# pyannote/pyannote-audio

Hardware: NVIDIA H100
Metric: audio-hours/sec (RTF) community-1 diarization, 16kHz mono, 1/2/4/8 H100 (higher is better)
Workload: dtype f16 tensor-core trunk (f32 accumulate) + split-f16x3 tensor-core segmentation (f32-level accuracy) + f64 clustering

## Files before the change

### pyannote_audio_b200/csrc/emb_conv.cu

```cuda
#include "common.cuh"
#include "emb.cuh"
#include "tc_common.cuh"

namespace b200 {

constexpr int kWgThreads = 288;
constexpr int kTileM = 128;
constexpr int kRowHalo = 8;
constexpr int kMaxSlots = 16;

template <int N, bool WIDE = false, int MH = 1>
__device__ __forceinline__ void conv_epilogue(const float* acc, const ConvParams& p, size_t row, int w0) {
  const int lane = threadIdx.x & 31;
  const int c0 = 2 * (lane & 3) + (WIDE ? (int)blockIdx.y * N : 0);
#pragma unroll
  for (int m = 0; m < MH; ++m)
#pragma unroll
  for (int i = 0; i < 2; ++i) {
    const int w = w0 + 64 * m + ((threadIdx.x >> 5) & 3) * 16 + (lane >> 2) + 8 * i;
    if (w >= p.W_out) continue;
    const size_t pix = (row * p.W_out + w) * (size_t)(WIDE ? p.C_out : N);
    __half2 res[N / 8];
    if (N <= 128 && p.residual) {
#pragma unroll
// ... 28 lines not shown
  const int wt = blockIdx.x % p.tiles_w;
  const int bh = blockIdx.x / p.tiles_w;
  const int cchunks = p.C_in / CK;

  if (threadIdx.x == 0) {
    for (uint32_t s = 0; s < p.nstages; ++s) { mbar_init(bar_full + 8 * s, 1); mbar_init(bar_empty + 8 * s, 2); }
    asm volatile("fence.mbarrier_init.release.cluster;" ::: "memory");
  }
  __syncthreads();

  if (warp == 8) {
    if ((threadIdx.x & 31) == 0) {
      prefetch_tensormap(&tmA);
      prefetch_tensormap(&tmB);
      const int h = bh % p.H_out, b = bh / p.H_out;
      const int w_base = wt * kTileM * p.stride - p.pad, h_base = h * p.stride - p.pad;
      uint32_t stage = 0, phase = 0;
      for (int kh = 0; kh < p.taps_h; ++kh)
        for (int kw = 0; kw < p.taps_w; ++kw)
          for (int cc = 0; cc < cchunks; ++cc) {
            mbar_wait(bar_empty + 8 * stage, phase ^ 1);
            mbar_expect_tx(bar_full + 8 * stage, p.a_tx + p.b_bytes);
            const uint32_t sa = stage0 + stage * stage_bytes;
            tma_load_4d(&tmA, bar_full + 8 * stage, sa, cc * CK, w_base + kw, h_base + kh, b);
            tma_load_3d(&tmB, bar_full + 8 * stage, sa + p.a_bytes, cc * CK, WIDE ? (int)blockIdx.y * N : 0,
                        kh * p.taps_w + kw);
            if (++stage == p.nstages) { stage = 0; phase ^= 1; }
          }
    }
    return;
  }

  const int wg = warp >> 2;
  constexpr uint32_t row_bytes = CK * 2;
  float acc[N / 2];
#pragma unroll
  for (int i = 0; i < N / 2; ++i) acc[i] = 0.f;
  const int kblocks = p.taps_h * p.taps_w * cchunks;
  uint32_t stage = 0, phase = 0, prev = 0;
  for (int kb = 0; kb < kblocks; ++kb) {
    mbar_wait(bar_full + 8 * stage, phase);
    const uint32_t st = stage0 + stage * stage_bytes;
    const uint32_t sa = st + (uint32_t)wg * 64u * row_bytes, sb = st + p.a_bytes;
    wg_fence();
    const uint64_t ad = wg_desc(sa, row_bytes), bd = wg_desc(sb, row_bytes);
#pragma unroll
    for (int k = 0; k < CK / 16; ++k) Wgmma<N>::mma(acc, ad + 2 * k, bd + 2 * k);
    wg_commit();
    wg_wait<1>();
    if (kb > 0 && (threadIdx.x & 127) == 0) mbar_arrive(bar_empty + 8 * prev);
    prev = stage;
    if (++stage == p.nstages) { stage = 0; phase ^= 1; }
  }
  wg_wait<0>();
  conv_epilogue<N, WIDE>(acc, p, (size_t)bh, wt * kTileM + wg * 64);
}

template <int N>
__device__ __forceinline__ void row_taps_c32(float (&acc)[2][N / 2], uint32_t sa, uint32_t wts) {
  constexpr uint32_t row_bytes = 64;
  const int warp = threadIdx.x >> 5, lane = threadIdx.x & 31;
#pragma unroll
  for (int kw = 0; kw < 3; ++kw) {
    uint32_t af[2][2][4];
#pragma unroll
    for (int m = 0; m < 2; ++m)
#pragma unroll
      for (int k = 0; k < 2; ++k) {
        const uint32_t row = (uint32_t)(m * 64 + (warp & 3) * 16 + (lane & 15) + kw);
        const uint32_t chunk = (uint32_t)(2 * k + (lane >> 4)) ^ ((row >> 1) & 3u);
        ldsm_x4(af[m][k], sa + row * row_bytes + chunk * 16u);
      }
    wg_fence();
    const uint64_t bd = wg_desc(wts + kw * N * row_bytes, row_bytes);
#pragma unroll
    for (int k = 0; k < 2; ++k)
#pragma unroll
      for (int m = 0; m < 2; ++m) WgmmaRS<N>::mma(acc[m], af[m][k], bd + 2 * k);
    wg_commit();
    wg_wait<0>();
  }
}

template <int N, int CK>
__global__ void __launch_bounds__(kWgThreads, N == 32 ? 2 : 1)
conv_row_kernel(const __grid_constant__ CUtensorMap tmA, const __grid_constant__ CUtensorMap tmB, ConvParams p) {
  constexpr uint32_t row_bytes = CK * 2;
  constexpr uint32_t b_tap_bytes = N * row_bytes;
  extern __shared__ uint8_t smem_raw[];
  const uint32_t base = (smem_u32(smem_raw) + 1023u) & ~1023u;
  const uint32_t bar_w = base, bar_full = base + 8, bar_empty = base + 8 + 8 * kMaxSlots;
  const uint32_t wts = base + 1024;
  const uint32_t slot0 = wts + 9 * b_tap_bytes;
  const uint32_t nslots = p.nstages;
  const int warp = threadIdx.x >> 5;

  if (threadIdx.x == 0) {
    mbar_init(bar_w, 1);
    for (uint32_t s = 0; s < nslots; ++s) { mbar_init(bar_full + 8 * s, 1); mbar_init(bar_empty + 8 * s, 3); }
    asm volatile("fence.mbarrier_init.release.cluster;" ::: "memory");
  }
  __syncthreads();

  if (warp == 8) {
    if ((threadIdx.x & 31) == 0) {
      prefetch_tensormap(&tmA);
      prefetch_tensormap(&tmB);
      mbar_expect_tx(bar_w, 9 * b_tap_bytes);
      for (int kh = 0; kh < 3; ++kh) tma_load_3d(&tmB, bar_w, wts + 3 * kh * b_tap_bytes, 0, 0, 3 * kh);
      uint32_t s = 0;
      for (int u = blockIdx.x; u < p.num_tiles; u += gridDim.x) {
        const int wt = u % p.tiles_w, t = u / p.tiles_w;
        const int h0 = (t % p.bands) * p.band, b = t / p.bands;
        const int n = min(p.band, p.H_out - h0);
        for (int r = 0; r < n + 2; ++r, ++s) {
          const uint32_t slot = s % nslots;
          mbar_wait(bar_empty + 8 * slot, ((s / nslots) & 1) ^ 1);
          mbar_expect_tx(bar_full + 8 * slot, p.a_tx);
          tma_load_4d(&tmA, bar_full + 8 * slot, slot0 + slot * p.a_bytes, 0, wt * kTileM - 1, h0 - 1 + r, b);
        }
      }
    }
    return;
  }

  const int wg = __shfl_sync(0xffffffffu, warp >> 2, 0);
  mbar_wait(bar_w, 0);
  uint32_t s = 0;
  int item = 0;
  for (int u = blockIdx.x; u < p.num_tiles; u += gridDim.x) {
    const int wt = u % p.tiles_w, t = u / p.tiles_w;
    const int h0 = (t % p.bands) * p.band, b = t / p.bands;
    const int n = min(p.band, p.H_out - h0);
    for (int j = 0; j < n; ++j, ++item) {
      if ((item & 1) != wg) continue;
      float acc[2][N / 2];
#pragma unroll
      for (int m = 0; m < 2; ++m)
#pragma unroll
        for (int i = 0; i < N / 2; ++i) {
          acc[m][i] = 0.f;
          asm volatile("" : "+f"(acc[m][i]));
        }
#pragma unroll
      for (int kh = 0; kh < 3; ++kh) {
        const uint32_t q = s + j + kh, slot = q % nslots;
        mbar_wait(bar_full + 8 * slot, (q / nslots) & 1);
        const uint32_t sa = slot0 + slot * p.a_bytes;
        if constexpr (CK == 32) {
          row_taps_c32<N>(acc, sa, wts + 3 * kh * b_tap_bytes);
        } else {
          wg_fence();
#pragma unroll
          for (int kw = 0; kw < 3; ++kw) {
            const uint64_t bd = wg_desc(wts + (3 * kh + kw) * b_tap_bytes, row_bytes);
#pragma unroll
            for (int m = 0; m < 2; ++m) {
              const uint64_t ad = wg_desc(sa + (uint32_t)(m * 64 + kw) * row_bytes, row_bytes);
#pragma unroll
              for (int k = 0; k < CK / 16; ++k) Wgmma<N>::mma(acc[m], ad + 2 * k, bd + 2 * k);
            }
          }
          wg_commit();
        }
      }
      wg_wait<0>();
      if ((threadIdx.x & 127) == 0)
#pragma unroll
        for (int kh = 0; kh < 3; ++kh)
          mbar_arrive_n(bar_empty + 8 * ((s + j + kh) % nslots), 1 + (j == 0 ? 2 - kh : 0) + (j == n - 1 ? kh : 0));
      const size_t row = (size_t)b * p.H_out + h0 + j;
#pragma unroll
      for (int m = 0; m < 2; ++m) conv_epilogue<N>(acc[m], p, row, wt * kTileM + m * 64);
    }
    s += n + 2;
  }
}

struct BlockRowPlan {
  static constexpr uint32_t kTapBytes = 32 * 64;
  static constexpr uint32_t kSlotBytes = 9 * 1024;
  static constexpr uint32_t kInTx = (kTileM + kRowHalo) * 64;
  static constexpr uint32_t kInSlots = 4, kMidSlots = 4;
  static constexpr size_t kSmem = 2048 + 2 * 9 * kTapBytes + (kInSlots + kMidSlots) * kSlotBytes;
  static_assert(kInTx <= kSlotBytes && kSmem <= 113 * 1024, "block row plan");
};
constexpr int kStripW = kTileM - 2;

struct BlockParams {
  int H, W, tiles_w, band, bands, num_tiles;
  const float* bias1;
  const float* bias2;
  __half* out;
};

__device__ __forceinline__ void st_shared_u32(uint32_t a, uint32_t v) {
  asm volatile("st.shared.b32 [%0], %1;" ::"r"(a), "r"(v) : "memory");
}
__device__ __forceinline__ uint32_t ld_shared_u32(uint32_t a) {
  uint32_t v;
  asm volatile("ld.shared.b32 %0, [%1];" : "=r"(v) : "r"(a) : "memory");
  return v;
}
__device__ __forceinline__ uint32_t h2_bits(__half2 h) { return *reinterpret_cast<uint32_t*>(&h); }

__global__ void __launch_bounds__(kWgThreads, 2)
block_row_kernel(const __grid_constant__ CUtensorMap tmA, const __grid_constant__ CUtensorMap tmW1,
                 const __grid_constant__ CUtensorMap tmW2, BlockParams p) {
  using P = BlockRowPlan;
  constexpr uint32_t NI = P::kInSlots, NM = P::kMidSlots;
  extern __shared__ uint8_t smem_raw[];
  const uint32_t base = (smem_u32(smem_raw) + 1023u) & ~1023u;
  const uint32_t bar_w = base, in_full = base + 8, in_empty = in_full + 8 * NI;
  const uint32_t mid_full = in_empty + 8 * NI, mid_empty = mid_full + 8 * NM;
  const uint32_t w1 = base + 1024, w2 = w1 + 9 * P::kTapBytes;
  const uint32_t in0 = w2 + 9 * P::kTapBytes, mid0 = in0 + NI * P::kSlotBytes;
  const int warp = threadIdx.x >> 5, lane = threadIdx.x & 31;

  if (threadIdx.x == 0) {
    mbar_init(bar_w, 1);
    for (uint32_t s = 0; s < NI; ++s) { mbar_init(in_full + 8 * s, 1); mbar_init(in_empty + 8 * s, 4); }
    for (uint32_t s = 0; s < NM; ++s) { mbar_init(mid_full + 8 * s, 128); mbar_init(mid_empty + 8 * s, 3); }
    asm volatile("fence.mbarrier_init.release.cluster;" ::: "memory");
  }
  __syncthreads();

  if (warp == 8) {
    if (lane == 0) {
      prefetch_tensormap(&tmA);
      prefetch_tensormap(&tmW1);
      prefetch_tensormap(&tmW2);
      mbar_expect_tx(bar_w, 18 * P::kTapBytes);
      for (int kh = 0; kh < 3; ++kh) {
        tma_load_3d(&tmW1, bar_w, w1 + 3 * kh * P::kTapBytes, 0, 0, 3 * kh);
        tma_load_3d(&tmW2, bar_w, w2 + 3 * kh * P::kTapBytes, 0, 0, 3 * kh);
      }
      uint32_t s = 0;
      for (int u = blockIdx.x; u < p.num_tiles; u += gridDim.x) {
        const int wt = u % p.tiles_w, t = u / p.tiles_w;
        const int h0 = (t % p.bands) * p.band, b = t / p.bands;
        const int n = min(p.band, p.H - h0);
        for (int r = 0; r < n + 4; ++r, ++s) {
          const uint32_t slot = s % NI;
          mbar_wait(in_empty + 8 * slot, ((s / NI) & 1) ^ 1);
          mbar_expect_tx(in_full + 8 * slot, P::kInTx);
          tma_load_4d(&tmA, in_full + 8 * slot, in0 + slot * P::kSlotBytes, 0, wt * kStripW - 2, h0 - 2 + r, b);
        }
      }
    }
    return;
  }

  const int wg = __shfl_sync(0xffffffffu, warp >> 2, 0);
  const bool leader = (threadIdx.x & 127) == 0;
  const int c0 = 2 * (lane & 3);
  float2 bias[4];
#pragma unroll
  for (int j = 0; j < 4; ++j) bias[j] = __ldg(reinterpret_cast<const float2*>((wg ? p.bias2 : p.bias1) + 8 * j + c0));
  mbar_wait(bar_w, 0);
  uint32_t s = 0, mq = 0;
  for (int u = blockIdx.x; u < p.num_tiles; u += gridDim.x) {
    const int wt = u % p.tiles_w, t = u / p.tiles_w;
    const int h0 = (t % p.bands) * p.band, b = t / p.bands;
    const int n = min(p.band, p.H - h0);
    const int w0 = wt * kStripW;
    const int rows = wg == 0 ? n + 2 : n;
    for (int j = 0; j < rows; ++j) {
      float acc[2][16];
#pragma unroll
      for (int m = 0; m < 2; ++m)
#pragma unroll
        for (int i = 0; i < 16; ++i) {
          acc[m][i] = 0.f;
          asm volatile("" : "+f"(acc[m][i]));
        }
      if (wg == 0) {
#pragma unroll
        for (int kh = 0; kh < 3; ++kh) {
          const uint32_t q = s + j + kh, slot = q % NI;
          mbar_wait(in_full + 8 * slot, (q / NI) & 1);
          row_taps_c32<32>(acc, in0 + slot * P::kSlotBytes, w1 + 3 * kh * P::kTapBytes);
        }
        if (leader)
#pragma unroll
          for (int kh = 0; kh < 3; ++kh) {
            const int k = j + kh;
            const bool no_res = (k < 2 || k >= n + 2) && j == min(k, n + 1);
// ... 297 lines not shown
      for (int q = 0; q < 8; ++q) {
        const ulonglong2 w4 = wk[q];
        ffma2(acc2[2 * q], xk, w4.x);
        ffma2(acc2[2 * q + 1], xk, w4.y);
      }
    }
    __half2 o[16];
#pragma unroll
    for (int c = 0; c < 16; ++c) {
      float a0, a1;
      unpack2(acc2[c], a0, a1);
      o[c] = __floats2half2_rn(fmaxf(a0, 0.f), fmaxf(a1, 0.f));
    }
    uint4* op = reinterpret_cast<uint4*>(out + (((size_t)b * kMel + h) * T0 + t) * 32);
    const uint4* src = reinterpret_cast<const uint4*>(o);
#pragma unroll
    for (int i = 0; i < 4; ++i) op[i] = src[i];
  }
}

typedef CUresult (*PFN_encodeTiled)(CUtensorMap*, CUtensorMapDataType, cuuint32_t, void*, const cuuint64_t*,
                                    const cuuint64_t*, const cuuint32_t*, const cuuint32_t*, CUtensorMapInterleave,
                                    CUtensorMapSwizzle, CUtensorMapL2promotion, CUtensorMapFloatOOBfill);

static PFN_encodeTiled get_encode() {
  static PFN_encodeTiled fn = nullptr;
  if (!fn) {
    void* ptr = nullptr;
    cudaDriverEntryPointQueryResult qres;
    if (cudaGetDriverEntryPoint("cuTensorMapEncodeTiled", &ptr, cudaEnableDefault, &qres) == cudaSuccess &&
        qres == cudaDriverEntryPointSuccess)
      fn = reinterpret_cast<PFN_encodeTiled>(ptr);
  }
  return fn;
}

int encode_f16_map(CUtensorMap* tm, int rank, const void* ptr, const cuuint64_t* dims, const cuuint64_t* strides,
                   const cuuint32_t* box, const cuuint32_t* estr, CUtensorMapSwizzle swizzle, const char* what) {
  PFN_encodeTiled enc = get_encode();
  B200_CHECK(enc != nullptr, B200_ERR_CUDA, "cuTensorMapEncodeTiled not available from the driver");
  const cuuint32_t ones[5] = {1, 1, 1, 1, 1};
  CUresult r = enc(tm, CU_TENSOR_MAP_DATA_TYPE_FLOAT16, (cuuint32_t)rank, const_cast<void*>(ptr), dims, strides, box,
                   estr ? estr : ones, CU_TENSOR_MAP_INTERLEAVE_NONE, swizzle, CU_TENSOR_MAP_L2_PROMOTION_L2_256B,
                   CU_TENSOR_MAP_FLOAT_OOB_FILL_NONE);
  B200_CHECK(r == CUDA_SUCCESS, B200_ERR_CUDA, "cuTensorMapEncodeTiled(%s) failed: %d", what, (int)r);
  return B200_OK;
}

int conv_forward(const ConvLayer& L, const __half* in, const __half* residual, __half* out, int B, int H_in, int W_in,
                 int relu, int impl, int num_sms, cudaStream_t stream) {
  ConvParams p{};
  p.B = B; p.H_in = H_in; p.W_in = W_in; p.C_in = L.C_in; p.C_out = L.C_out;
  p.taps_h = L.ksize; p.taps_w = L.ksize; p.stride = L.stride; p.pad = L.ksize / 2;
  p.H_out = (H_in + 2 * p.pad - L.ksize) / L.stride + 1;
  p.W_out = (W_in + 2 * p.pad - L.ksize) / L.stride + 1;
  p.relu = relu; p.bias = L.bias; p.residual = residual; p.out = out;
  p.Ck = (L.C_in >= 64) ? 64 : 32;
  p.swizzle = (p.Ck == 64) ? 128 : 64;
  p.tiles_w = ceil_div(p.W_out, kTileM);
  p.num_tiles = B * p.H_out * p.tiles_w;
  B200_CHECK(L.C_in % p.Ck == 0 && (L.C_out == 32 || L.C_out == 64 || L.C_out == 128 ||
                                    (L.C_out % 256 == 0 && L.C_out <= 1024 && p.Ck == 64)),
             B200_ERR_STATE, "conv %d -> %d channels unsupported", L.C_in, L.C_out);
  const int n_tile = std::min(L.C_out, 256);
  B200_CHECK(impl >= 0 && impl <= 2, B200_ERR_INVALID,
             "conv_impl %d unknown (0 = CUDA cores, 1 = tensor cores, 2 = tensor cores, one weight tap per stage)", impl);

  if (impl == 0) {
    const size_t total = (size_t)B * p.H_out * p.W_out * (L.C_out / 8);
    conv_simt_kernel<<<(unsigned)((total + 255) / 256), 256, 0, stream>>>(in, L.w, p);
    B200_CUDA_OK(cudaGetLastError());
    return B200_OK;
  }

  const bool rows = impl == 1 && L.ksize == 3 && L.stride == 1 && L.C_in == p.Ck && L.C_out == L.C_in;
  const bool chunk_rows =
      impl == 1 && L.ksize == 3 && L.stride == 1 && L.C_out == L.C_in && (L.C_out == 128 || L.C_out == 256);
  p.a_rows = rows || chunk_rows ? kTileM + kRowHalo : kTileM;
  p.a_tx = p.a_rows * p.Ck * 2;
  p.a_bytes = (p.a_tx + 1023u) & ~1023u;
  size_t smem;
  int ctas = 0;
  if (rows) {
    const int per_sm = L.C_out == 32 ? 2 : 1;
    const size_t budget = per_sm == 2 ? 113u * 1024 : 227u * 1024;
    const size_t fixed = 2048 + (size_t)9 * L.C_out * p.Ck * 2;
    p.nstages = (uint32_t)std::min<size_t>(kMaxSlots, (budget - fixed) / p.a_bytes);
    B200_CHECK(p.nstages >= 6, B200_ERR_STATE, "conv %d -> %d: row ring too shallow", L.C_in, L.C_out);
    smem = fixed + (size_t)p.nstages * p.a_bytes;
    ctas = per_sm * num_sms;
    const int strips = B * p.tiles_w;
    const int nbands = std::min(p.H_out, ceil_div(ctas, strips));
    p.band = ceil_div(p.H_out, nbands);
    p.bands = ceil_div(p.H_out, p.band);
    p.num_tiles = strips * p.bands;
  } else if (chunk_rows) {
    p.band = L.C_out == 256 ? ChunkRowPlan<256>::kRows : ChunkRowPlan<128>::kRows;
    p.bands = ceil_div(p.H_out, p.band);
    p.num_tiles = B * p.bands * p.tiles_w;
    smem = L.C_out == 256 ? ChunkRowPlan<256>::kSmem : ChunkRowPlan<128>::kSmem;
    ctas = num_sms;
  } else {
    p.b_bytes = (uint32_t)(n_tile * p.Ck * 2);
    const uint32_t budget = n_tile == 256 ? 200u * 1024 : 100u * 1024;
    p.nstages = std::min(budget / (p.a_bytes + p.b_bytes), 8u);
    B200_CHECK(p.nstages >= 2, B200_ERR_STATE, "conv %d -> %d: shared memory plan too shallow", L.C_in, L.C_out);
    smem = 1024 + 1024 + (size_t)p.nstages * (p.a_bytes + p.b_bytes);
  }
  const CUtensorMapSwizzle swz = p.swizzle == 128 ? CU_TENSOR_MAP_SWIZZLE_128B : CU_TENSOR_MAP_SWIZZLE_64B;
  CUtensorMap tmA, tmB;
  int rc;
  {
    const cuuint64_t dims[4] = {(cuuint64_t)L.C_in, (cuuint64_t)W_in, (cuuint64_t)H_in, (cuuint64_t)B};
    const cuuint64_t strides[3] = {(cuuint64_t)L.C_in * 2, (cuuint64_t)W_in * L.C_in * 2,
                                   (cuuint64_t)H_in * W_in * L.C_in * 2};
    const cuuint32_t box[4] = {(cuuint32_t)p.Ck, (cuuint32_t)(p.a_rows * L.stride), 1, 1};
    const cuuint32_t estr[4] = {1, (cuuint32_t)L.stride, 1, 1};
    if ((rc = encode_f16_map(&tmA, 4, in, dims, strides, box, estr, swz, "A"))) return rc;
  }
  {
    const cuuint64_t dims[3] = {(cuuint64_t)L.C_in, (cuuint64_t)L.C_out, (cuuint64_t)(L.ksize * L.ksize)};
    const cuuint64_t strides[2] = {(cuuint64_t)L.C_in * 2, (cuuint64_t)L.C_out * L.C_in * 2};
    const cuuint32_t box[3] = {(cuuint32_t)p.Ck, (cuuint32_t)n_tile, rows ? 3u : 1u};
    if ((rc = encode_f16_map(&tmB, 3, L.w, dims, strides, box, nullptr, swz, "B"))) return rc;
  }
  auto launch = [&](auto kernel) -> int {
    B200_CUDA_OK(cudaFuncSetAttribute(kernel, cudaFuncAttributeMaxDynamicSharedMemorySize, (int)smem));
    const dim3 grid((unsigned)(ctas ? std::min(p.num_tiles, ctas) : p.num_tiles), (unsigned)(L.C_out / n_tile));
    kernel<<<grid, kWgThreads, smem, stream>>>(tmA, tmB, p);
    B200_CUDA_OK(cudaGetLastError());
    return B200_OK;
  };
  if (rows) return p.Ck == 32 ? launch(conv_row_kernel<32, 32>) : launch(conv_row_kernel<64, 64>);
  if (chunk_rows) return L.C_out == 256 ? launch(conv_chunk_row_kernel<256>) : launch(conv_chunk_row_kernel<128>);
  if (p.Ck == 32) {
    switch (L.C_out) {
      case 32: return launch(conv_tc_kernel<32, 32>);
      case 64: return launch(conv_tc_kernel<64, 32>);
      default: return launch(conv_tc_kernel<128, 32>);
    }
  }
  switch (L.C_out) {
    case 32: return launch(conv_tc_kernel<32, 64>);
    case 64: return launch(conv_tc_kernel<64, 64>);
    case 128: return launch(conv_tc_kernel<128, 64>);
    case 256: return launch(conv_tc_kernel<256, 64>);
    default: return launch(conv_tc_kernel<256, 64, true>);
  }
}

bool block_fused(const BlockWeights& Bw, int impl) {
  return impl == 1 && !Bw.has_shortcut && Bw.conv1.stride == 1 && Bw.conv1.ksize == 3 && Bw.conv2.ksize == 3 &&
         Bw.conv1.C_in == 32 && Bw.conv1.C_out == 32 && Bw.conv2.C_in == 32 && Bw.conv2.C_out == 32;
}

int block_forward(const BlockWeights& Bw, const __half* in, __half* out, int B, int H, int W, int num_sms,
                  cudaStream_t stream) {
  B200_CHECK(block_fused(Bw, 1), B200_ERR_STATE, "block %d -> %d (stride %d) has no fused kernel", Bw.conv1.C_in,
             Bw.conv1.C_out, Bw.conv1.stride);
  B200_CHECK(in != out, B200_ERR_INVALID, "fused block: output must not alias the input");
  BlockParams p{};
  p.H = H; p.W = W; p.bias1 = Bw.conv1.bias; p.bias2 = Bw.conv2.bias; p.out = out;
  p.tiles_w = ceil_div(W, kStripW);
  const int ctas = 2 * num_sms;
  const int strips = B * p.tiles_w;
  const int nbands = std::min(H, ceil_div(ctas, strips));
  p.band = ceil_div(H, nbands);
  p.bands = ceil_div(H, p.band);
  p.num_tiles = strips * p.bands;
  CUtensorMap tmA, tmW1, tmW2;
  int rc;
  {
    const cuuint64_t dims[4] = {32, (cuuint64_t)W, (cuuint64_t)H, (cuuint64_t)B};
    const cuuint64_t strides[3] = {64, (cuuint64_t)W * 64, (cuuint64_t)H * W * 64};
    const cuuint32_t box[4] = {32, kTileM + kRowHalo, 1, 1};
    if ((rc = encode_f16_map(&tmA, 4, in, dims, strides, box, nullptr, CU_TENSOR_MAP_SWIZZLE_64B, "block A"))) return rc;
  }
  {
    const cuuint64_t dims[3] = {32, 32, 9};
    const cuuint64_t strides[2] = {64, 32 * 64};
    const cuuint32_t box[3] = {32, 32, 3};
    if ((rc = encode_f16_map(&tmW1, 3, Bw.conv1.w, dims, strides, box, nullptr, CU_TENSOR_MAP_SWIZZLE_64B, "block W1")))
      return rc;
    if ((rc = encode_f16_map(&tmW2, 3, Bw.conv2.w, dims, strides, box, nullptr, CU_TENSOR_MAP_SWIZZLE_64B, "block W2")))
      return rc;
  }
  const size_t smem = BlockRowPlan::kSmem;
  B200_CUDA_OK(cudaFuncSetAttribute(block_row_kernel, cudaFuncAttributeMaxDynamicSharedMemorySize, (int)smem));
  block_row_kernel<<<(unsigned)std::min(p.num_tiles, ctas), kWgThreads, smem, stream>>>(tmA, tmW1, tmW2, p);
  B200_CUDA_OK(cudaGetLastError());
  return B200_OK;
}

int conv1_forward(const float* fbank, const float* fmean, const int* frame0, const float* w, const float* bias,
                  __half* out, int B, int T0, cudaStream_t stream) {
  dim3 grid(B, ceil_div(T0, kC1Tile));
  conv1_kernel<<<grid, kC1Tile, 0, stream>>>(fbank, fmean, frame0, w, bias, out, T0);
  B200_CUDA_OK(cudaGetLastError());
  return B200_OK;
}

}
```

### pyannote_audio_b200/csrc/tc_common.cuh

```cuda
#pragma once
#include "common.cuh"
#include <cuda.h>

namespace b200 {

__device__ __forceinline__ uint32_t smem_u32(const void* p) {
  return static_cast<uint32_t>(__cvta_generic_to_shared(p));
}
__device__ __forceinline__ void mbar_init(uint32_t bar, uint32_t count) {
  asm volatile("mbarrier.init.shared::cta.b64 [%0], %1;" ::"r"(bar), "r"(count));
}
__device__ __forceinline__ void mbar_expect_tx(uint32_t bar, uint32_t bytes) {
  asm volatile("mbarrier.arrive.expect_tx.shared::cta.b64 _, [%0], %1;" ::"r"(bar), "r"(bytes) : "memory");
}
__device__ __forceinline__ void mbar_arrive(uint32_t bar) {
  asm volatile("mbarrier.arrive.shared::cta.b64 _, [%0];" ::"r"(bar) : "memory");
}
__device__ __forceinline__ void mbar_arrive_n(uint32_t bar, uint32_t count) {
  asm volatile("mbarrier.arrive.shared::cta.b64 _, [%0], %1;" ::"r"(bar), "r"(count) : "memory");
}
__device__ __forceinline__ void mbar_wait(uint32_t bar, uint32_t parity) {
  asm volatile(
      "{\n\t"
      ".reg .pred p;\n\t"
      "WAIT_%=:\n\t"
      "mbarrier.try_wait.parity.shared::cta.b64 p, [%0], %1;\n\t"
      "@p bra DONE_%=;\n\t"
      "bra WAIT_%=;\n\t"
      "DONE_%=:\n\t"
      "}" ::"r"(bar), "r"(parity)
      : "memory");
}
__device__ __forceinline__ void tma_load_4d(const CUtensorMap* tm, uint32_t bar, uint32_t dst, int c0, int c1, int c2,
                                            int c3) {
  asm volatile(
      "cp.async.bulk.tensor.4d.shared::cluster.global.mbarrier::complete_tx::bytes [%0], [%1, {%3, %4, %5, %6}], [%2];"
      ::"r"(dst), "l"(reinterpret_cast<uint64_t>(tm)), "r"(bar), "r"(c0), "r"(c1), "r"(c2), "r"(c3)
      : "memory");
}
__device__ __forceinline__ void tma_load_3d(const CUtensorMap* tm, uint32_t bar, uint32_t dst, int c0, int c1, int c2) {
  asm volatile(
      "cp.async.bulk.tensor.3d.shared::cluster.global.mbarrier::complete_tx::bytes [%0], [%1, {%3, %4, %5}], [%2];"
      ::"r"(dst), "l"(reinterpret_cast<uint64_t>(tm)), "r"(bar), "r"(c0), "r"(c1), "r"(c2)
      : "memory");
}
__device__ __forceinline__ void tma_load_2d(const CUtensorMap* tm, uint32_t bar, uint32_t dst, int c0, int c1) {
  asm volatile(
      "cp.async.bulk.tensor.2d.shared::cluster.global.mbarrier::complete_tx::bytes [%0], [%1, {%3, %4}], [%2];"
      ::"r"(dst), "l"(reinterpret_cast<uint64_t>(tm)), "r"(bar), "r"(c0), "r"(c1)
      : "memory");
}
__device__ __forceinline__ void prefetch_tensormap(const CUtensorMap* tm) {
  asm volatile("prefetch.tensormap [%0];" ::"l"(reinterpret_cast<uint64_t>(tm)) : "memory");
}

__device__ __forceinline__ uint64_t wg_desc(uint32_t saddr, uint32_t swizzle_bytes) {
  const uint64_t layout = swizzle_bytes == 128 ? 1u : 2u;
  return (uint64_t)((saddr & 0x3FFFFu) >> 4) | ((uint64_t)1 << 16) | ((uint64_t)((8u * swizzle_bytes) >> 4) << 32) |
         (layout << 62);
}
__device__ __forceinline__ void ldsm_x4(uint32_t* r, uint32_t saddr) {
  asm volatile("ldmatrix.sync.aligned.m8n8.x4.shared.b16 {%0, %1, %2, %3}, [%4];"
               : "=r"(r[0]), "=r"(r[1]), "=r"(r[2]), "=r"(r[3])
               : "r"(saddr)
               : "memory");
}
__device__ __forceinline__ void wg_fence() { asm volatile("wgmma.fence.sync.aligned;" ::: "memory"); }
__device__ __forceinline__ void wg_commit() { asm volatile("wgmma.commit_group.sync.aligned;" ::: "memory"); }
template <int N>
__device__ __forceinline__ void wg_wait() { asm volatile("wgmma.wait_group.sync.aligned %0;" ::"n"(N) : "memory"); }

template <int N>
struct Wgmma;
template <>
struct Wgmma<32> {
  __device__ __forceinline__ static void mma(float* d, uint64_t a, uint64_t b) {
    asm volatile(
        "wgmma.mma_async.sync.aligned.m64n32k16.f32.f16.f16 "
        "{%0, %1, %2, %3, %4, %5, %6, %7, %8, %9, %10, %11, %12, %13, %14, %15}, %16, %17, 1, 1, 1, 0, 0;"
        : "+f"(d[0]), "+f"(d[1]), "+f"(d[2]), "+f"(d[3]), "+f"(d[4]), "+f"(d[5]), "+f"(d[6]), "+f"(d[7]), "+f"(d[8]), "+f"(d[9]), "+f"(d[10]), "+f"(d[11]), "+f"(d[12]), "+f"(d[13]), "+f"(d[14]), "+f"(d[15])
        : "l"(a), "l"(b));
  }
};
template <>
struct Wgmma<64> {
  __device__ __forceinline__ static void mma(float* d, uint64_t a, uint64_t b) {
    asm volatile(
        "wgmma.mma_async.sync.aligned.m64n64k16.f32.f16.f16 "
        "{%0, %1, %2, %3, %4, %5, %6, %7, %8, %9, %10, %11, %12, %13, %14, %15, %16, %17, %18, %19, %20, %21, %22, %23, %24, %25, %26, %27, %28, %29, %30, %31}, %32, %33, 1, 1, 1, 0, 0;"
        : "+f"(d[0]), "+f"(d[1]), "+f"(d[2]), "+f"(d[3]), "+f"(d[4]), "+f"(d[5]), "+f"(d[6]), "+f"(d[7]), "+f"(d[8]), "+f"(d[9]), "+f"(d[10]), "+f"(d[11]), "+f"(d[12]), "+f"(d[13]), "+f"(d[14]), "+f"(d[15]), "+f"(d[16]), "+f"(d[17]), "+f"(d[18]), "+f"(d[19]), "+f"(d[20]), "+f"(d[21]), "+f"(d[22]), "+f"(d[23]), "+f"(d[24]), "+f"(d[25]), "+f"(d[26]), "+f"(d[27]), "+f"(d[28]), "+f"(d[29]), "+f"(d[30]), "+f"(d[31])
        : "l"(a), "l"(b));
  }
};
template <>
struct Wgmma<128> {
  __device__ __forceinline__ static void mma(float* d, uint64_t a, uint64_t b) {
    asm volatile(
        "wgmma.mma_async.sync.aligned.m64n128k16.f32.f16.f16 "
        "{%0, %1, %2, %3, %4, %5, %6, %7, %8, %9, %10, %11, %12, %13, %14, %15, %16, %17, %18, %19, %20, %21, %22, %23, %24, %25, %26, %27, %28, %29, %30, %31, %32, %33, %34, %35, %36, %37, %38, %39, %40, %41, %42, %43, %44, %45, %46, %47, %48, %49, %50, %51, %52, %53, %54, %55, %56, %57, %58, %59, %60, %61, %62, %63}, %64, %65, 1, 1, 1, 0, 0;"
        : "+f"(d[0]), "+f"(d[1]), "+f"(d[2]), "+f"(d[3]), "+f"(d[4]), "+f"(d[5]), "+f"(d[6]), "+f"(d[7]), "+f"(d[8]), "+f"(d[9]), "+f"(d[10]), "+f"(d[11]), "+f"(d[12]), "+f"(d[13]), "+f"(d[14]), "+f"(d[15]), "+f"(d[16]), "+f"(d[17]), "+f"(d[18]), "+f"(d[19]), "+f"(d[20]), "+f"(d[21]), "+f"(d[22]), "+f"(d[23]), "+f"(d[24]), "+f"(d[25]), "+f"(d[26]), "+f"(d[27]), "+f"(d[28]), "+f"(d[29]), "+f"(d[30]), "+f"(d[31]), "+f"(d[32]), "+f"(d[33]), "+f"(d[34]), "+f"(d[35]), "+f"(d[36]), "+f"(d[37]), "+f"(d[38]), "+f"(d[39]), "+f"(d[40]), "+f"(d[41]), "+f"(d[42]), "+f"(d[43]), "+f"(d[44]), "+f"(d[45]), "+f"(d[46]), "+f"(d[47]), "+f"(d[48]), "+f"(d[49]), "+f"(d[50]), "+f"(d[51]), "+f"(d[52]), "+f"(d[53]), "+f"(d[54]), "+f"(d[55]), "+f"(d[56]), "+f"(d[57]), "+f"(d[58]), "+f"(d[59]), "+f"(d[60]), "+f"(d[61]), "+f"(d[62]), "+f"(d[63])
        : "l"(a), "l"(b));
  }
};
template <>
struct Wgmma<256> {
  __device__ __forceinline__ static void mma(float* d, uint64_t a, uint64_t b) {
    asm volatile(
        "wgmma.mma_async.sync.aligned.m64n256k16.f32.f16.f16 "
        "{%0, %1, %2, %3, %4, %5, %6, %7, %8, %9, %10, %11, %12, %13, %14, %15, %16, %17, %18, %19, %20, %21, %22, %23, %24, %25, %26, %27, %28, %29, %30, %31, %32, %33, %34, %35, %36, %37, %38, %39, %40, %41, %42, %43, %44, %45, %46, %47, %48, %49, %50, %51, %52, %53, %54, %55, %56, %57, %58, %59, %60, %61, %62, %63, %64, %65, %66, %67, %68, %69, %70, %71, %72, %73, %74, %75, %76, %77, %78, %79, %80, %81, %82, %83, %84, %85, %86, %87, %88, %89, %90, %91, %92, %93, %94, %95, %96, %97, %98, %99, %100, %101, %102, %103, %104, %105, %106, %107, %108, %109, %110, %111, %112, %113, %114, %115, %116, %117, %118, %119, %120, %121, %122, %123, %124, %125, %126, %127}, %128, %129, 1, 1, 1, 0, 0;"
        : "+f"(d[0]), "+f"(d[1]), "+f"(d[2]), "+f"(d[3]), "+f"(d[4]), "+f"(d[5]), "+f"(d[6]), "+f"(d[7]), "+f"(d[8]), "+f"(d[9]), "+f"(d[10]), "+f"(d[11]), "+f"(d[12]), "+f"(d[13]), "+f"(d[14]), "+f"(d[15]), "+f"(d[16]), "+f"(d[17]), "+f"(d[18]), "+f"(d[19]), "+f"(d[20]), "+f"(d[21]), "+f"(d[22]), "+f"(d[23]), "+f"(d[24]), "+f"(d[25]), "+f"(d[26]), "+f"(d[27]), "+f"(d[28]), "+f"(d[29]), "+f"(d[30]), "+f"(d[31]), "+f"(d[32]), "+f"(d[33]), "+f"(d[34]), "+f"(d[35]), "+f"(d[36]), "+f"(d[37]), "+f"(d[38]), "+f"(d[39]), "+f"(d[40]), "+f"(d[41]), "+f"(d[42]), "+f"(d[43]), "+f"(d[44]), "+f"(d[45]), "+f"(d[46]), "+f"(d[47]), "+f"(d[48]), "+f"(d[49]), "+f"(d[50]), "+f"(d[51]), "+f"(d[52]), "+f"(d[53]), "+f"(d[54]), "+f"(d[55]), "+f"(d[56]), "+f"(d[57]), "+f"(d[58]), "+f"(d[59]), "+f"(d[60]), "+f"(d[61]), "+f"(d[62]), "+f"(d[63]), "+f"(d[64]), "+f"(d[65]), "+f"(d[66]), "+f"(d[67]), "+f"(d[68]), "+f"(d[69]), "+f"(d[70]), "+f"(d[71]), "+f"(d[72]), "+f"(d[73]), "+f"(d[74]), "+f"(d[75]), "+f"(d[76]), "+f"(d[77]), "+f"(d[78]), "+f"(d[79]), "+f"(d[80]), "+f"(d[81]), "+f"(d[82]), "+f"(d[83]), "+f"(d[84]), "+f"(d[85]), "+f"(d[86]), "+f"(d[87]), "+f"(d[88]), "+f"(d[89]), "+f"(d[90]), "+f"(d[91]), "+f"(d[92]), "+f"(d[93]), "+f"(d[94]), "+f"(d[95]), "+f"(d[96]), "+f"(d[97]), "+f"(d[98]), "+f"(d[99]), "+f"(d[100]), "+f"(d[101]), "+f"(d[102]), "+f"(d[103]), "+f"(d[104]), "+f"(d[105]), "+f"(d[106]), "+f"(d[107]), "+f"(d[108]), "+f"(d[109]), "+f"(d[110]), "+f"(d[111]), "+f"(d[112]), "+f"(d[113]), "+f"(d[114]), "+f"(d[115]), "+f"(d[116]), "+f"(d[117]), "+f"(d[118]), "+f"(d[119]), "+f"(d[120]), "+f"(d[121]), "+f"(d[122]), "+f"(d[123]), "+f"(d[124]), "+f"(d[125]), "+f"(d[126]), "+f"(d[127])
        : "l"(a), "l"(b));
  }
};

template <int N>
struct WgmmaRS;
template <>
struct WgmmaRS<32> {
  __device__ __forceinline__ static void mma(float* d, const uint32_t* a, uint64_t b) {
    asm volatile(
        "wgmma.mma_async.sync.aligned.m64n32k16.f32.f16.f16 "
        "{%0, %1, %2, %3, %4, %5, %6, %7, %8, %9, %10, %11, %12, %13, %14, %15}, {%16, %17, %18, %19}, %20, 1, 1, 1, 0;"
        : "+f"(d[0]), "+f"(d[1]), "+f"(d[2]), "+f"(d[3]), "+f"(d[4]), "+f"(d[5]), "+f"(d[6]), "+f"(d[7]), "+f"(d[8]), "+f"(d[9]), "+f"(d[10]), "+f"(d[11]), "+f"(d[12]), "+f"(d[13]), "+f"(d[14]), "+f"(d[15])
        : "r"(a[0]), "r"(a[1]), "r"(a[2]), "r"(a[3]), "l"(b));
  }
};
template <>
struct WgmmaRS<64> {
  __device__ __forceinline__ static void mma(float* d, const uint32_t* a, uint64_t b) {
    asm volatile(
        "wgmma.mma_async.sync.aligned.m64n64k16.f32.f16.f16 "
        "{%0, %1, %2, %3, %4, %5, %6, %7, %8, %9, %10, %11, %12, %13, %14, %15, %16, %17, %18, %19, %20, %21, %22, %23, %24, %25, %26, %27, %28, %29, %30, %31}, {%32, %33, %34, %35}, %36, 1, 1, 1, 0;"
        : "+f"(d[0]), "+f"(d[1]), "+f"(d[2]), "+f"(d[3]), "+f"(d[4]), "+f"(d[5]), "+f"(d[6]), "+f"(d[7]), "+f"(d[8]), "+f"(d[9]), "+f"(d[10]), "+f"(d[11]), "+f"(d[12]), "+f"(d[13]), "+f"(d[14]), "+f"(d[15]), "+f"(d[16]), "+f"(d[17]), "+f"(d[18]), "+f"(d[19]), "+f"(d[20]), "+f"(d[21]), "+f"(d[22]), "+f"(d[23]), "+f"(d[24]), "+f"(d[25]), "+f"(d[26]), "+f"(d[27]), "+f"(d[28]), "+f"(d[29]), "+f"(d[30]), "+f"(d[31])
        : "r"(a[0]), "r"(a[1]), "r"(a[2]), "r"(a[3]), "l"(b));
  }
};
template <>
// ... 25 lines not shown
```

Baseline: 1.659.

## Stage conv row residual and output through shared memory with TMA loads and stores

The row conv kernel now has its producer warp TMA-load the residual tile into a per-warpgroup shared buffer a few slots behind the input ring. The epilogue reads the residual and writes the result into that swizzled tile, then issues a TMA bulk store in place of per-thread global loads and stores. Bias is hoisted into registers, and the ring depth becomes a compile-time plan per channel count. This aims to cut uncoalesced epilogue global traffic, at the cost of shared memory taken from the input ring and extra barrier synchronisation.

```diff
diff --git a/pyannote_audio_b200/csrc/emb_conv.cu b/pyannote_audio_b200/csrc/emb_conv.cu
--- a/pyannote_audio_b200/csrc/emb_conv.cu
+++ b/pyannote_audio_b200/csrc/emb_conv.cu
@@ -134,22 +134,57 @@
   }
 }
 
+__device__ __forceinline__ void st_shared_u32(uint32_t a, uint32_t v) {
+  asm volatile("st.shared.b32 [%0], %1;" ::"r"(a), "r"(v) : "memory");
+}
+__device__ __forceinline__ uint32_t ld_shared_u32(uint32_t a) {
+  uint32_t v;
+  asm volatile("ld.shared.b32 %0, [%1];" : "=r"(v) : "r"(a) : "memory");
+  return v;
+}
+__device__ __forceinline__ uint32_t h2_bits(__half2 h) { return *reinterpret_cast<uint32_t*>(&h); }
+__device__ __forceinline__ void named_bar_sync(int id) { asm volatile("bar.sync %0, 128;" ::"r"(id) : "memory"); }
+
+template <int N>
+struct RowPlan {
+  static constexpr uint32_t kRowBytes = N * 2;
+  static constexpr uint32_t kTapBytes = N * kRowBytes;
+  static constexpr uint32_t kInTx = (kTileM + kRowHalo) * kRowBytes;
+  static constexpr uint32_t kSlotBytes = (kInTx + 1023u) & ~1023u;
+  static constexpr uint32_t kTileBytes = kTileM * kRowBytes;
+  static constexpr uint32_t kSlots = N == 64 ? 7 : 8;
+  static constexpr int kResLag = (int)kSlots - 2;
+  static constexpr int kCtasPerSm = N == 32 ? 2 : 1;
+  static constexpr size_t kBudget = N == 32 ? 113u * 1024 : 227u * 1024;
+  static constexpr size_t kSmem = 2048 + 9 * kTapBytes + 2 * kTileBytes + kSlots * kSlotBytes;
+  static_assert(N == 32 || N == 64, "row kernel: 32 or 64 channels");
+  static_assert(kSlots >= 6 && kSlots <= kMaxSlots, "row ring: four slots in use and two ahead");
+  static_assert(kSmem <= kBudget && kSmem + kSlotBytes > kBudget, "row plan: every slot that fits");
+};
+
 template <int N, int CK>
 __global__ void __launch_bounds__(kWgThreads, N == 32 ? 2 : 1)
-conv_row_kernel(const __grid_constant__ CUtensorMap tmA, const __grid_constant__ CUtensorMap tmB, ConvParams p) {
-  constexpr uint32_t row_bytes = CK * 2;
-  constexpr uint32_t b_tap_bytes = N * row_bytes;
+conv_row_kernel(const __grid_constant__ CUtensorMap tmA, const __grid_constant__ CUtensorMap tmB,
+                const __grid_constant__ CUtensorMap tmR, const __grid_constant__ CUtensorMap tmO, ConvParams p) {
+  using P = RowPlan<N>;
+  static_assert(CK == N, "row kernel: one channel chunk");
+  constexpr uint32_t row_bytes = P::kRowBytes;
+  constexpr uint32_t b_tap_bytes = P::kTapBytes;
+  constexpr uint32_t nslots = P::kSlots;
   extern __shared__ uint8_t smem_raw[];
   const uint32_t base = (smem_u32(smem_raw) + 1023u) & ~1023u;
   const uint32_t bar_w = base, bar_full = base + 8, bar_empty = base + 8 + 8 * kMaxSlots;
+  const uint32_t tile_full = base + 512, tile_empty = base + 528;
   const uint32_t wts = base + 1024;
-  const uint32_t slot0 = wts + 9 * b_tap_bytes;
-  const uint32_t nslots = p.nstages;
+  const uint32_t tile0 = wts + 9 * b_tap_bytes;
+  const uint32_t slot0 = tile0 + 2 * P::kTileBytes;
+  const bool has_res = p.residual != nullptr;
   const int warp = threadIdx.x >> 5;
 
   if (threadIdx.x == 0) {
     mbar_init(bar_w, 1);
     for (uint32_t s = 0; s < nslots; ++s) { mbar_init(bar_full + 8 * s, 1); mbar_init(bar_empty + 8 * s, 3); }
+    for (uint32_t s = 0; s < 2; ++s) { mbar_init(tile_full + 8 * s, 1); mbar_init(tile_empty + 8 * s, 1); }
     asm volatile("fence.mbarrier_init.release.cluster;" ::: "memory");
   }
   __syncthreads();
@@ -158,25 +193,45 @@
     if ((threadIdx.x & 31) == 0) {
       prefetch_tensormap(&tmA);
       prefetch_tensormap(&tmB);
+      if (has_res) prefetch_tensormap(&tmR);
       mbar_expect_tx(bar_w, 9 * b_tap_bytes);
       for (int kh = 0; kh < 3; ++kh) tma_load_3d(&tmB, bar_w, wts + 3 * kh * b_tap_bytes, 0, 0, 3 * kh);
       uint32_t s = 0;
+      uint32_t k = 0;
       for (int u = blockIdx.x; u < p.num_tiles; u += gridDim.x) {
         const int wt = u % p.tiles_w, t = u / p.tiles_w;
         const int h0 = (t % p.bands) * p.band, b = t / p.bands;
         const int n = min(p.band, p.H_out - h0);
+        auto stage_residual = [&](int j) {
+          const uint32_t tile = k & 1, use = k >> 1;
+          mbar_wait(tile_empty + 8 * tile, (use & 1) ^ 1);
+          mbar_expect_tx(tile_full + 8 * tile, P::kTileBytes);
+          tma_load_4d(&tmR, tile_full + 8 * tile, tile0 + tile * P::kTileBytes, 0, wt * kTileM, h0 + j, b);
+          ++k;
+        };
         for (int r = 0; r < n + 2; ++r, ++s) {
           const uint32_t slot = s % nslots;
           mbar_wait(bar_empty + 8 * slot, ((s / nslots) & 1) ^ 1);
-          mbar_expect_tx(bar_full + 8 * slot, p.a_tx);
-          tma_load_4d(&tmA, bar_full + 8 * slot, slot0 + slot * p.a_bytes, 0, wt * kTileM - 1, h0 - 1 + r, b);
-        }
+          mbar_expect_tx(bar_full + 8 * slot, P::kInTx);
+          tma_load_4d(&tmA, bar_full + 8 * slot, slot0 + slot * P::kSlotBytes, 0, wt * kTileM - 1, h0 - 1 + r, b);
+          if (has_res && r >= P::kResLag) stage_residual(r - P::kResLag);
+        }
+        if (has_res)
+          for (int j = max(0, n + 2 - P::kResLag); j < n; ++j) stage_residual(j);
       }
     }
     return;
   }
 
   const int wg = __shfl_sync(0xffffffffu, warp >> 2, 0);
+  const int lane = threadIdx.x & 31;
+  const bool leader = (threadIdx.x & 127) == 0;
+  const uint32_t tile = tile0 + wg * P::kTileBytes;
+  const int c0 = 2 * (lane & 3);
+  float2 bias[N / 8];
+#pragma unroll
+  for (int j = 0; j < N / 8; ++j) bias[j] = __ldg(reinterpret_cast<const float2*>(p.bias + 8 * j + c0));
+  if (leader) prefetch_tensormap(&tmO);
   mbar_wait(bar_w, 0);
   uint32_t s = 0;
   int item = 0;
@@ -198,7 +253,7 @@
       for (int kh = 0; kh < 3; ++kh) {
         const uint32_t q = s + j + kh, slot = q % nslots;
         mbar_wait(bar_full + 8 * slot, (q / nslots) & 1);
-        const uint32_t sa = slot0 + slot * p.a_bytes;
+        const uint32_t sa = slot0 + slot * P::kSlotBytes;
         if constexpr (CK == 32) {
           row_taps_c32<N>(acc, sa, wts + 3 * kh * b_tap_bytes);
         } else {
@@ -217,16 +272,50 @@
         }
       }
       wg_wait<0>();
-      if ((threadIdx.x & 127) == 0)
+      if (leader)
 #pragma unroll
         for (int kh = 0; kh < 3; ++kh)
           mbar_arrive_n(bar_empty + 8 * ((s + j + kh) % nslots), 1 + (j == 0 ? 2 - kh : 0) + (j == n - 1 ? kh : 0));
-      const size_t row = (size_t)b * p.H_out + h0 + j;
-#pragma unroll
-      for (int m = 0; m < 2; ++m) conv_epilogue<N>(acc[m], p, row, wt * kTileM + m * 64);
+      if (has_res) {
+        mbar_wait(tile_full + 8 * wg, (item >> 1) & 1);
+      } else {
+        if (leader) bulk_wait_read<0>();
+        named_bar_sync(1 + wg);
+      }
+#pragma unroll
+      for (int m = 0; m < 2; ++m)
+#pragma unroll
+        for (int i = 0; i < 2; ++i) {
+          const uint32_t px = m * 64 + (warp & 3) * 16 + (lane >> 2) + 8 * i;
+          const uint32_t swz = row_bytes == 128 ? px & 7u : (px >> 1) & 3u;
+#pragma unroll
+          for (int jj = 0; jj < N / 8; ++jj) {
+            const uint32_t ta = tile + px * row_bytes + ((jj ^ swz) << 4) + 2 * c0;
+            float a = acc[m][4 * jj + 2 * i] + bias[jj].x, d = acc[m][4 * jj + 2 * i + 1] + bias[jj].y;
+            if (has_res) {
+              const uint32_t rb = ld_shared_u32(ta);
+              const float2 r = __half22float2(*reinterpret_cast<const __half2*>(&rb));
+              a += r.x;
+              d += r.y;
+            }
+            if (p.relu) { a = fmaxf(a, 0.f); d = fmaxf(d, 0.f); }
+            st_shared_u32(ta, h2_bits(__floats2half2_rn(a, d)));
+          }
+        }
+      fence_proxy_async();
+      named_bar_sync(1 + wg);
+      if (leader) {
+        tma_store_4d(&tmO, tile, 0, wt * kTileM, h0 + j, b);
+        bulk_commit();
+        if (has_res) {
+          bulk_wait_read<0>();
+          mbar_arrive(tile_empty + 8 * wg);
+        }
+      }
     }
     s += n + 2;
   }
+  if (leader) bulk_wait<0>();
 }
 
 struct BlockRowPlan {
@@ -246,15 +335,6 @@
   __half* out;
 };
 
-__device__ __forceinline__ void st_shared_u32(uint32_t a, uint32_t v) {
-  asm volatile("st.shared.b32 [%0], %1;" ::"r"(a), "r"(v) : "memory");
-}
-__device__ __forceinline__ uint32_t ld_shared_u32(uint32_t a) {
-  uint32_t v;
-  asm volatile("ld.shared.b32 %0, [%1];" : "=r"(v) : "r"(a) : "memory");
-  return v;
-}
-__device__ __forceinline__ uint32_t h2_bits(__half2 h) { return *reinterpret_cast<uint32_t*>(&h); }
 
 __global__ void __launch_bounds__(kWgThreads, 2)
 block_row_kernel(const __grid_constant__ CUtensorMap tmA, const __grid_constant__ CUtensorMap tmW1,
@@ -718,12 +798,8 @@
   size_t smem;
   int ctas = 0;
   if (rows) {
-    const int per_sm = L.C_out == 32 ? 2 : 1;
-    const size_t budget = per_sm == 2 ? 113u * 1024 : 227u * 1024;
-    const size_t fixed = 2048 + (size_t)9 * L.C_out * p.Ck * 2;
-    p.nstages = (uint32_t)std::min<size_t>(kMaxSlots, (budget - fixed) / p.a_bytes);
-    B200_CHECK(p.nstages >= 6, B200_ERR_STATE, "conv %d -> %d: row ring too shallow", L.C_in, L.C_out);
-    smem = fixed + (size_t)p.nstages * p.a_bytes;
+    const int per_sm = L.C_out == 32 ? RowPlan<32>::kCtasPerSm : RowPlan<64>::kCtasPerSm;
+    smem = L.C_out == 32 ? RowPlan<32>::kSmem : RowPlan<64>::kSmem;
     ctas = per_sm * num_sms;
     const int strips = B * p.tiles_w;
     const int nbands = std::min(p.H_out, ceil_div(ctas, strips));
@@ -760,6 +836,20 @@
     const cuuint32_t box[3] = {(cuuint32_t)p.Ck, (cuuint32_t)n_tile, rows ? 3u : 1u};
     if ((rc = encode_f16_map(&tmB, 3, L.w, dims, strides, box, nullptr, swz, "B"))) return rc;
   }
+  if (rows) {
+    CUtensorMap tmR{}, tmO;
+    const cuuint64_t dims[4] = {(cuuint64_t)L.C_out, (cuuint64_t)p.W_out, (cuuint64_t)p.H_out, (cuuint64_t)B};
+    const cuuint64_t strides[3] = {(cuuint64_t)L.C_out * 2, (cuuint64_t)p.W_out * L.C_out * 2,
+                                   (cuuint64_t)p.H_out * p.W_out * L.C_out * 2};
+    const cuuint32_t box[4] = {(cuuint32_t)L.C_out, (cuuint32_t)kTileM, 1, 1};
+    if (residual && (rc = encode_f16_map(&tmR, 4, residual, dims, strides, box, nullptr, swz, "residual"))) return rc;
+    if ((rc = encode_f16_map(&tmO, 4, out, dims, strides, box, nullptr, swz, "out"))) return rc;
+    auto kernel = p.Ck == 32 ? conv_row_kernel<32, 32> : conv_row_kernel<64, 64>;
+    B200_CUDA_OK(cudaFuncSetAttribute(kernel, cudaFuncAttributeMaxDynamicSharedMemorySize, (int)smem));
+    kernel<<<(unsigned)std::min(p.num_tiles, ctas), kWgThreads, smem, stream>>>(tmA, tmB, tmR, tmO, p);
+    B200_CUDA_OK(cudaGetLastError());
+    return B200_OK;
+  }
   auto launch = [&](auto kernel) -> int {
     B200_CUDA_OK(cudaFuncSetAttribute(kernel, cudaFuncAttributeMaxDynamicSharedMemorySize, (int)smem));
     const dim3 grid((unsigned)(ctas ? std::min(p.num_tiles, ctas) : p.num_tiles), (unsigned)(L.C_out / n_tile));
@@ -767,7 +857,6 @@
     B200_CUDA_OK(cudaGetLastError());
     return B200_OK;
   };
-  if (rows) return p.Ck == 32 ? launch(conv_row_kernel<32, 32>) : launch(conv_row_kernel<64, 64>);
   if (chunk_rows) return L.C_out == 256 ? launch(conv_chunk_row_kernel<256>) : launch(conv_chunk_row_kernel<128>);
   if (p.Ck == 32) {
     switch (L.C_out) {
diff --git a/pyannote_audio_b200/csrc/tc_common.cuh b/pyannote_audio_b200/csrc/tc_common.cuh
--- a/pyannote_audio_b200/csrc/tc_common.cuh
+++ b/pyannote_audio_b200/csrc/tc_common.cuh
@@ -53,6 +53,17 @@
 __device__ __forceinline__ void prefetch_tensormap(const CUtensorMap* tm) {
   asm volatile("prefetch.tensormap [%0];" ::"l"(reinterpret_cast<uint64_t>(tm)) : "memory");
 }
+__device__ __forceinline__ void tma_store_4d(const CUtensorMap* tm, uint32_t src, int c0, int c1, int c2, int c3) {
+  asm volatile("cp.async.bulk.tensor.4d.global.shared::cta.bulk_group [%0, {%2, %3, %4, %5}], [%1];"
+               ::"l"(reinterpret_cast<uint64_t>(tm)), "r"(src), "r"(c0), "r"(c1), "r"(c2), "r"(c3)
+               : "memory");
+}
+__device__ __forceinline__ void fence_proxy_async() { asm volatile("fence.proxy.async.shared::cta;" ::: "memory"); }
+__device__ __forceinline__ void bulk_commit() { asm volatile("cp.async.bulk.commit_group;" ::: "memory"); }
+template <int N>
+__device__ __forceinline__ void bulk_wait_read() { asm volatile("cp.async.bulk.wait_group.read %0;" ::"n"(N) : "memory"); }
+template <int N>
+__device__ __forceinline__ void bulk_wait() { asm volatile("cp.async.bulk.wait_group %0;" ::"n"(N) : "memory"); }
 
 __device__ __forceinline__ uint64_t wg_desc(uint32_t saddr, uint32_t swizzle_bytes) {
   const uint64_t layout = swizzle_bytes == 128 ? 1u : 2u;
```

New measurement: 1.745, median of 6. 5.2% higher.
